# yhao-wang/DenseRetrievalToolkits

Measured on AMD Instinct MI355X. Metric: queries/sec@top-1000, 10Mx768 corpus (BASELINE: passages encoded/sec + queries/sec@top-1000, 10Mx768 corpus, 1/2/4/8 GPU), higher is better.
Workload: dtype bf16

## Files before the change

denseretrievaltoolkits_amd/_native.py:

```python
from __future__ import annotations

import ctypes
import os
import threading

import torch

from .build_native import LIB_PATH

DRT_OK = 0
DRT_EINVAL = -1
ROW_STATS_LEN = 34

_lock = threading.Lock()
_lib = None

c_i32 = ctypes.c_int32
c_i64 = ctypes.c_int64
c_sz = ctypes.c_size_t
c_vp = ctypes.c_void_p
c_f32 = ctypes.c_float
c_u64 = ctypes.c_uint64

_SIGNATURES = [
    ("drt_version", ctypes.c_char_p, []),
    ("drt_ip_topk_workspace", c_sz, [c_i64, c_i64, c_i32, c_i32]),
    ("drt_ip_topk_bf16", c_i32, [c_vp, c_i64, c_vp, c_i64, c_i32, c_i32, c_i64, c_vp, c_vp, c_vp, c_vp, c_sz, c_vp]),
    ("drt_ip_topk_resolve_workspace", c_sz, [c_i64, c_i64, c_i32]),
    ("drt_ip_topk_resolve", c_i32, [c_vp, c_i64, c_vp, c_i64, c_i32, c_i32, c_i64, c_vp, c_vp, c_vp, c_vp, c_sz,
                                    c_vp, c_vp]),
    ("drt_topk_merge", c_i32, [c_vp, c_vp, c_i64, c_i32, c_i32, c_i32, c_vp, c_vp, c_vp]),
    ("drt_ip_topk_sample_rank", c_i32, [c_i32]),
    ("drt_ip_topk_dist_workspace", c_sz, [c_i64, c_i64, c_i64, c_i32, c_i32]),
    ("drt_ip_topk_dist_sample", c_i32, [c_vp, c_i64, c_vp, c_i64, c_i64, c_i32, c_i32, c_vp, c_vp, c_sz, c_vp]),
    ("drt_ip_topk_dist_tau", c_i32, [c_vp, c_i64, c_i32, c_i32, c_vp, c_vp]),
    ("drt_ip_topk_dist_filter", c_i32, [c_vp, c_i64, c_vp, c_i64, c_i64, c_i32, c_i32, c_i64, c_vp, c_vp, c_vp,
                                        c_sz, c_vp]),
    ("drt_ip_topk_dist_filter_chunks", c_i32, [c_vp, c_i64, c_vp, c_i64, c_i64, c_i32, c_i32, c_i64, c_vp, c_vp,
                                               c_vp, c_i32, c_vp, c_sz, c_vp]),
    ("drt_ip_topk_dist_filter_lists", c_i32, [c_vp, c_i64, c_vp, c_i64, c_i64, c_i32, c_i32, c_i64, c_vp, c_i32,
                                              c_vp, c_vp, c_vp, c_sz, c_vp]),
    ("drt_ip_topk_dist_filter_lists_at", c_i32, [c_vp, c_i64, c_vp, c_i64, c_i64, c_i32, c_i32, c_i64, c_vp,
                                                 c_i32, c_i64, c_vp, c_vp, c_vp, c_sz, c_vp]),
    ("drt_topk_merge_packed", c_i32, [c_vp, c_i64, c_i32, c_i32, c_i64, c_vp, c_vp, c_vp, c_vp]),
    ("drt_topk_merge_packed_cert", c_i32, [c_vp, c_i64, c_i32, c_i32, c_i32, c_i64, c_vp, c_vp, c_vp, c_vp]),
    ("drt_topk_merge_packed_capped", c_i32, [c_vp, c_i64, c_i32, c_i32, c_i32, c_i32, c_i64, c_vp, c_vp, c_vp,
                                             c_vp]),
    ("drt_row_stats_bf16", c_i32, [c_vp, c_i64, c_i32, c_vp, c_i32, c_vp]),
    ("drt_refine_width", c_i32, [c_i32]),
    ("drt_ip_topk_exact_bf16", c_i32, [c_vp, c_i64, c_vp, c_i64, c_i32, c_i32, c_i64, c_vp, c_vp, c_vp, c_vp, c_vp,
                                       c_sz, c_vp]),
    ("drt_hit_metrics_i8", c_i32, [c_vp, c_i64, c_i64, c_vp, c_i32, c_vp, c_vp]),
    ("drt_answer_match_i32", c_i32, [c_vp, c_i32, c_vp, c_vp, c_i64, c_i64, c_i64, c_vp, c_vp, c_i32, c_i32, c_vp,
                                     c_vp, c_vp]),
# ... 121 lines not shown
```

denseretrievaltoolkits_amd/csrc/search.hip:

```cpp
#include <algorithm>
#include <cmath>
#include <vector>

#include "drt_common.h"
#include "profile.h"

namespace drt {

constexpr int kScanThreads = 256;
constexpr int kQueriesPerWG = 128;
constexpr int kHitCap = 1024;
constexpr int kCntStride = 32;

enum { SCAN_FILTER = 0, SCAN_DENSE = 1, SCAN_TOPR = 2 };
constexpr int kTopRL = 4;

struct ScanArgs {
  const __bf16* Q;
  int64_t nq;
  int64_t ldq;
  const __bf16* P;
  int64_t ldp;
  int64_t row0;
  int64_t nrows;
  int64_t rstride;
  const float* tau;
  uint32_t* counts;
  void* out;
  int64_t cap;
  int64_t exp_hits;
  uint32_t row_base;
};

__device__ __forceinline__ void glds16(const void* gsrc, uint32_t lds_addr) {
  uint32_t keep;
  asm volatile(
      "s_mov_b32 %0, m0\n\t"
      "s_mov_b32 m0, %2\n\t"
      "s_nop 0\n\t"
      "global_load_lds_dwordx4 %1, off\n\t"
      "s_mov_b32 m0, %0"
      : "=&s"(keep)
      : "v"(gsrc), "s"(lds_addr)
      : "memory");
}

__device__ __forceinline__ void glds16_nt(const void* gsrc, uint32_t lds_addr) {
// ... 448 lines not shown
__global__ __launch_bounds__(512, 1) void ip_scan16r_kernel(ScanArgs a) {
  constexpr int NW = 8;
  using C = Scan16Cfg<D, NW>;
  constexpr int PD = C::NBUF;
  __shared__ __attribute__((aligned(16))) char smem[C::LDS_BYTES];

  const int tid = threadIdx.x;
  const int wave = __builtin_amdgcn_readfirstlane(tid >> 6);
  const int lane = tid & 63;
  const int r = lane & 15;
  const int kq = lane >> 4;
  uint64_t* hk = (uint64_t*)(smem + C::HIT_KEY_OFF) + wave * kWaveSeg;
  uint8_t* hq = (uint8_t*)(smem + C::HIT_Q_OFF) + wave * kWaveSeg;

  const int64_t qbase = (int64_t)blockIdx.y * kQueriesPerWG;
  const int ntiles = (int)((a.nrows + kT16 - 1) / kT16);
  const uint32_t nrows = (uint32_t)a.nrows;
  const int t0 = blockIdx.x;
  const int tstep = gridDim.x;
  const int my_tiles = t0 < ntiles ? (ntiles - 1 - t0) / tstep + 1 : 0;
  if (my_tiles == 0) return;
  const int partial_tile = (a.nrows & (kT16 - 1)) != 0 ? ntiles - 1 : -1;
  const uint32_t ring = lds_addr_of(smem);
  const int64_t tile_stride = (int64_t)tstep * kT16 * a.ldp * 2;
  const char* next_base = (const char*)(a.P + (int64_t)t0 * kT16 * a.ldp);

  const int64_t qw = qbase + wave * 16;
  const int64_t qg = qw + r;
  const bool qok = qg < a.nq;
  const int64_t qs = qok ? qg : 0;
  bf16x8 qf[C::KS];
#pragma unroll
  for (int s = 0; s < C::KS; ++s) qf[s] = *(const bf16x8*)(a.Q + qs * a.ldq + s * 32 + kq * 8);
  float tau = __builtin_nanf("");
  {
    const float tv = a.tau[qs];
    tau = qok ? tv : tau;
  }
  if (!qok) {
#pragma unroll
    for (int s = 0; s < C::KS; ++s) qf[s] = (bf16x8){};
  }
#pragma unroll
  for (int s = 0; s < C::KS; ++s) asm volatile("" ::"v"(qf[s]));
  asm volatile("" ::"v"(tau));
  asm volatile("s_waitcnt vmcnt(0)" ::: "memory");

  LeanTile<D, NW> lt;
  lt.init(a, wave, lane);
#pragma unroll
  for (int p = 0; p < PD; ++p) {
    if (p < my_tiles) {
      const int tile = t0 + p * tstep;
      lt.template issue<NT>(a, ring + p * C::TILE_BYTES, next_base, tile == partial_tile, tile, wave, lane);
      next_base += tile_stride;
    }
  }
  if (wave >= NW / 2) __builtin_amdgcn_s_setprio(1);
  {
    const int last = my_tiles - 1 < PD - 1 ? my_tiles - 1 : PD - 1;
    wait_tiles_younger<C::GLDS_PER_WAVE>((int)last);
  }
  lds_barrier();

  const int sw = (r >> 1) & 7;
  int aoff[2];
#pragma unroll
  for (int m = 0; m < 2; ++m) aoff[m] = r * 128 + (((4 * m + kq) ^ sw) << 4);
  bf16x8 af[C::KS];
// ... 60 lines not shown
  };

  f32x4 accA, accB;
  uint32_t rbA = 0, rbB = 0;
  int buf = 0;
  auto iter = [&](int it, f32x4& acc, uint32_t& rb, const f32x4& prev, uint32_t rb_prev) {
    const int tile = t0 + it * tstep;
    if (it + PD <= my_tiles) {
      wait_vmcnt<C::GLDS_PER_WAVE * (PD - 2)>();
    } else if (it + 1 < my_tiles) {
      wait_tiles_younger<C::GLDS_PER_WAVE>(my_tiles - 1 - it - 1);
    }
    lds_barrier();
    if (it + PD < my_tiles) {
      const int ntile = tile + PD * tstep;
      lt.template issue<NT>(a, ring + buf * C::TILE_BYTES, next_base, ntile == partial_tile, ntile, wave, lane);
      next_base += tile_stride;
    }
    const int nslot = buf + 1 == C::NBUF ? 0 : buf + 1;
    mma_roll(acc, nslot);
    if (it > 0) epilogue(prev, rb_prev);
    rb = (uint32_t)tile * kT16 + 4 * kq;
    buf = nslot;
  };
  for (int it = 0; it < my_tiles; it += 2) {
    iter(it, accA, rbA, accB, rbB);
    if (it + 1 < my_tiles) iter(it + 1, accB, rbB, accA, rbA);
  }
  if (my_tiles & 1) epilogue(accA, rbA);
  else epilogue(accB, rbB);
  if (wcnt) wave_flush_hits(a, qw, hk, hq, wcnt, lane);
}

template <int D>
struct Scan32Cfg {
  static constexpr int KS = D / 32;
  static constexpr int RD = KS % 2 == 0 ? 2 : 1;
// ... 17 lines not shown
  constexpr int PD = NB - 1;
  constexpr int KS = C32::KS;
  constexpr int RD = C32::RD;
  constexpr int kSeg = kHitCap / NW;
  __shared__ __attribute__((aligned(16))) char smem[C32::LDS_BYTES];

  const int tid = threadIdx.x;
  const int wave = __builtin_amdgcn_readfirstlane(tid >> 6);
  const int lane = tid & 63;
  const int r = lane & 15;
  const int kq = lane >> 4;
  uint64_t* hk = (uint64_t*)(smem + C32::RING_BYTES) + wave * kSeg;
  uint8_t* hq = (uint8_t*)(smem + C32::RING_BYTES + kHitCap * 8) + wave * kSeg;

  const int64_t qbase = (int64_t)blockIdx.y * kQueriesPerWG32;
  const int ntiles = (int)((a.nrows + kT16 - 1) / kT16);
  const uint32_t nrows = (uint32_t)a.nrows;
  const int t0 = blockIdx.x;
  const int tstep = gridDim.x;
  const int my_tiles = t0 < ntiles ? (ntiles - 1 - t0) / tstep + 1 : 0;
  if (my_tiles == 0) return;
  const int partial_tile = (a.nrows & (kT16 - 1)) != 0 ? ntiles - 1 : -1;
  const uint32_t ring = lds_addr_of(smem);
  const int64_t tile_stride = (int64_t)tstep * kT16 * a.ldp * 2;
  const char* next_base = (const char*)(a.P + (int64_t)t0 * kT16 * a.ldp);

  const int64_t qw = qbase + wave * 32;
  bf16x8 qf0[KS], qf1[KS];
  float tau0, tau1;
  {
    const int64_t g0 = qw + r, g1 = qw + 16 + r;
    const bool ok0 = g0 < a.nq, ok1 = g1 < a.nq;
    const int64_t s0 = ok0 ? g0 : 0, s1 = ok1 ? g1 : 0;
#pragma unroll
    for (int s = 0; s < KS; ++s) {
      qf0[s] = *(const bf16x8*)(a.Q + s0 * a.ldq + s * 32 + kq * 8);
      qf1[s] = *(const bf16x8*)(a.Q + s1 * a.ldq + s * 32 + kq * 8);
    }
    const float v0 = a.tau[s0], v1 = a.tau[s1];
    tau0 = ok0 ? v0 : __builtin_nanf("");
// ... 6 lines not shown
#pragma unroll
      for (int s = 0; s < KS; ++s) qf1[s] = (bf16x8){};
    }
  }
#pragma unroll
  for (int s = 0; s < KS; ++s) asm volatile("" ::"v"(qf0[s]), "v"(qf1[s]));
  asm volatile("" ::"v"(tau0), "v"(tau1));
  asm volatile("s_waitcnt vmcnt(0)" ::: "memory");

  LeanTile<D, NW> lt;
  lt.init(a, wave, lane);
#pragma unroll
  for (int p = 0; p < PD; ++p) {
    if (p < my_tiles) {
      const int tile = t0 + p * tstep;
      lt.template issue<false>(a, ring + p * C::TILE_BYTES, next_base, tile == partial_tile, tile, wave, lane);
      next_base += tile_stride;
    }
  }
  if (wave >= NW / 2) __builtin_amdgcn_s_setprio(1);
  {
    const int last = my_tiles - 1 < PD - 1 ? my_tiles - 1 : PD - 1;
    wait_tiles_younger<C::GLDS_PER_WAVE>((int)last);
  }
  lds_barrier();

  const int sw = (r >> 1) & 7;
  int aoff[2];
#pragma unroll
  for (int m = 0; m < 2; ++m) aoff[m] = r * 128 + (((4 * m + kq) ^ sw) << 4);
  auto frag = [&](int slot, int s) -> bf16x8 {
// ... 43 lines not shown
    }
    lds_barrier();
    const bool do_dma = it + PD < my_tiles;
    const int ntile = tile + PD * tstep;
    const int pslot = buf == 0 ? NB - 1 : buf - 1;
    const int nslot = buf + 1 == NB ? 0 : buf + 1;
    acc0 = (f32x4){0.f, 0.f, 0.f, 0.f};
    acc1 = (f32x4){0.f, 0.f, 0.f, 0.f};
#pragma unroll
    for (int s = 0; s < KS; ++s) {
      acc0 = __builtin_amdgcn_mfma_f32_16x16x32_bf16(af[s % RD], qf0[s], acc0, 0, 0, 0);
      acc1 = __builtin_amdgcn_mfma_f32_16x16x32_bf16(af[s % RD], qf1[s], acc1, 0, 0, 0);
      af[s % RD] = s + RD < KS ? frag(buf, s + RD) : frag(nslot, s + RD - KS);
      __builtin_amdgcn_sched_barrier(0);
      if (s == KS / 4 && do_dma) {
        lt.template issue<false>(a, ring + pslot * C::TILE_BYTES, next_base, ntile == partial_tile, ntile, wave,
                                 lane);
        next_base += tile_stride;
      }
      __builtin_amdgcn_sched_barrier(0);
    }
    if (it > 0) epilogue(prev0, prev1, rb_prev);
    rb = (uint32_t)tile * kT16 + 4 * kq;
    buf = nslot;
  };
  f32x4 a0, a1, b0, b1;
  uint32_t rbA = 0, rbB = 0;
  for (int it = 0; it < my_tiles; it += 2) {
    iter(it, a0, a1, rbA, b0, b1, rbB);
    if (it + 1 < my_tiles) iter(it + 1, b0, b1, rbB, a0, a1, rbA);
  }
  if (my_tiles & 1) epilogue(a0, a1, rbA);
  else epilogue(b0, b1, rbB);
  if (wcnt) wave_flush_hits(a, qw, hk, hq, wcnt, lane);
}

enum { SEL_KEYS64 = 0, SEL_DENSE32 = 1 };
enum { SEL_TOPK = 0, SEL_KTH = 1 };
// ... 12 lines not shown
  int64_t n_in;
  int64_t cap;
  int64_t n_total;
  int k;
  int64_t nq;
  float* out_scores;
  int64_t* out_ids;
  int64_t ldo;
  int64_t id_offset;
  int32_t* status;
  const int32_t* qmap;
  float* tau;
  uint64_t* out_packed;
  bool global_tau;
  int k_cert;
};

template <int INPUT>
__device__ __forceinline__ uint64_t sel_load(const SelectArgs& a, int64_t q, int64_t j) {
  if (INPUT == SEL_KEYS64) return ((const uint64_t*)a.in)[q * a.in_stride + j];
  const uint32_t v = ((const uint32_t*)a.in)[q * a.in_stride + j];
  return ((uint64_t)v << 32) | (uint64_t)(uint32_t)j;
}

__device__ __forceinline__ float key_score(uint64_t x) { return desc_key_to_score((uint32_t)(x >> 32)); }

__device__ __forceinline__ int score_bin(float s, float smin, float scale) {
  if (scale == 0.0f) return 0;
  return hist_bin((s - smin) * scale, kSelBins, __builtin_signbit(s) ? 0 : kSelBins - 1);
}
// ... 409 lines not shown
  block_bitonic(buf, n2);

  const int64_t orow = a.qmap ? (int64_t)a.qmap[q] : q;
  if (a.out_packed) {
    uint64_t* op = a.out_packed + orow * (int64_t)(a.k + 1);
    for (int j = tid; j < a.k; j += kSelThreads) {
      if (j < kk_total) {
        const uint64_t x = buf[j];
        op[j] = (x & 0xFFFFFFFF00000000ull) | (uint64_t)(uint32_t)(a.id_offset + (int64_t)(x & 0xFFFFFFFFull));
      } else {
        op[j] = ~0ull;
      }
    }
    if (tid == 0) {
      const uint64_t nval = (uint64_t)(kk_total < a.k ? kk_total : a.k);
      op[a.k] = (nval << 32) | ((INPUT == SEL_KEYS64 && c_raw > a.cap) ? 1ull : 0ull) |
                (c_raw > (int64_t)a.k ? 2ull : 0ull);
    }
    return;
  }
  float* os = a.out_scores + orow * a.ldo;
  int64_t* oi = a.out_ids + orow * a.ldo;
  for (int j = tid; j < a.k; j += kSelThreads) {
    if (j < kk_total) {
      const uint64_t x = buf[j];
      os[j] = key_score(x);
      oi[j] = a.id_offset + (int64_t)(x & 0xFFFFFFFFull);
    } else {
      os[j] = kPadScore;
      oi[j] = -1;
    }
  }
  if (a.status && tid == 0) {
    int st = 0;
    if (INPUT == SEL_KEYS64) {
      if (c_raw > a.cap) st = 1;
      const int64_t kq = a.k_cert > 0 ? a.k_cert : a.k;
      if (!a.global_tau && c_raw < kq && c_raw < a.n_total) st = 1;
    }
    a.status[orow] = st;
  }
}

constexpr int kKthChunk = 4096;
constexpr int kKthThreads = 512;

__device__ __forceinline__ void block_bitonic_u32(uint32_t* buf, int n2) { block_sort<uint32_t, kKthThreads>(buf, n2); }

constexpr int kKthPer = kKthChunk / kKthThreads;
constexpr int kKthBins = 256;
constexpr int kKthSel = 1024;

__global__ __launch_bounds__(kKthThreads) void kth_partial_kernel(const uint32_t* in, int64_t stride, int64_t n,
                                                                  int r, uint32_t* part) {
  __shared__ __attribute__((aligned(16))) uint32_t buf[kKthChunk];
// ... 1717 lines not shown
static dim3 scan16_grid(int64_t nq, int64_t nrows) {
  const unsigned gy = (unsigned)((nq + kQueriesPerWG - 1) / kQueriesPerWG);
  const int64_t ntiles = (nrows + kT16 - 1) / kT16;
  int gx = scan_grid_x(ntiles);
  if (gy > 1 && ntiles >= 8) {
    const int cus = scan_grid_x((int64_t)1 << 40);
    const int share = std::max(8, (cus / (int)gy) & ~7);
    gx = (int)std::min<int64_t>(ntiles, share);
  }
  return dim3(gx, gy);
}

template <int D>
static int launch_scan_d(const ScanArgs& a, int mode, hipStream_t s) {
  if (a.nq == 0 || a.nrows == 0) return DRT_OK;
  const int64_t ntiles = (a.nrows + kT16 - 1) / kT16;
  const dim3 grid = scan16_grid(a.nq, a.nrows);
  const unsigned gy = grid.y;
  if (mode == SCAN_FILTER) {
    const double eh = a.exp_hits > 0 ? (double)a.exp_hits : (double)a.cap / 4.0;
    const bool dense_hits = eh * 256.0 / (double)a.nrows >= 0.35;
    if (D > 768 || a.row0 != 0 || a.rstride != 1) {
      if (dense_hits) hipLaunchKernelGGL((ip_scan16_kernel<D, SCAN_FILTER, 8, true>), grid, dim3(512), 0, s, a);
      else hipLaunchKernelGGL((ip_scan16_kernel<D, SCAN_FILTER, 8, false>), grid, dim3(512), 0, s, a);
    } else {
      if (D <= 768 && gy > 1) {
        const unsigned gy32 = (unsigned)((a.nq + kQueriesPerWG32 - 1) / kQueriesPerWG32);
        int gx32 = scan_grid_x(ntiles);
        if (gy32 > 1 && ntiles >= 8) {
          const int cus = scan_grid_x((int64_t)1 << 40);
          const int share = std::max(8, (cus / (int)gy32) & ~7);
          gx32 = (int)std::min<int64_t>(ntiles, share);
// ... 870 lines not shown
    a.tau = tau;
    a.counts = cnt;
    a.out = w + p.off_keys;
    a.cap = p.cap;
    a.exp_hits = p.sample ? std::max<int64_t>(1, target * rows / std::max<int64_t>(1, n_global)) : rows;
    a.row_base = (uint32_t)r0;
    const int rc = launch_scan(a, d, SCAN_FILTER, s, PROF_SCAN);
    if (rc) return rc;
  }
  sa.counts = cnt;
  sa.cap = p.cap;
  sa.n_total = n_local;
  return launch_select(sa, SEL_KEYS64, SEL_TOPK, s);
}

int drt_ip_topk_dist_filter_lists(const void* Q, int64_t nq, const void* P, int64_t n_local, int64_t n_global,
                                  int32_t d, int32_t k, int64_t id_offset, const uint32_t* lists, int32_t nlists,
                                  float* tau_out, uint64_t* packed, void* ws, size_t ws_bytes, void* stream) {
  const int32_t r = drt_ip_topk_sample_rank(k);
  return drt_ip_topk_dist_filter_lists_at(Q, nq, P, n_local, n_global, d, k, id_offset, lists, nlists,
                                          r > 0 ? nq * r : 0, tau_out, packed, ws, ws_bytes, stream);
}

int drt_ip_topk_dist_filter_lists_at(const void* Q, int64_t nq, const void* P, int64_t n_local, int64_t n_global,
                                     int32_t d, int32_t k, int64_t id_offset, const uint32_t* lists, int32_t nlists,
                                     int64_t lists_stride, float* tau_out, uint64_t* packed, void* ws,
                                     size_t ws_bytes, void* stream) {
  DRT_REQUIRE(valid_dist_dims(nq, n_local, n_global, d, k));
  DRT_REQUIRE(id_offset >= 0 && id_offset + n_local <= n_global);
  const int32_t r = drt_ip_topk_sample_rank(k);
// ... 135 lines not shown
```

denseretrievaltoolkits_amd/csrc/torch_ops.cpp:

```cpp
#include <vector>

#include <torch/library.h>
#include <ATen/ATen.h>
#include <c10/core/DeviceGuard.h>
#include <ATen/hip/impl/HIPStreamMasqueradingAsCUDA.h>

#include "drt.h"

namespace {

using at::Tensor;

void* stream_of(const Tensor& t) {
  return (void*)at::hip::getCurrentHIPStreamMasqueradingAsCUDA(t.device().index()).stream();
}

void check_rc(int rc, const char* what) {
  TORCH_CHECK_VALUE(rc != DRT_EINVAL, what, ": invalid argument (DRT_EINVAL)");
  TORCH_CHECK(rc == DRT_OK, what, ": HIP error ", rc);
}

void need_gpu(const Tensor& t, const char* name) {
  TORCH_CHECK(t.is_cuda(), "drt ops run on the GPU only (", name, " is on ", t.device(),
              "; no CPU fallback exists)");
// ... 370 lines not shown
  TORCH_CHECK_VALUE(tau.size(0) == q.size(0), "tau must hold one threshold per query");
  TORCH_CHECK_VALUE(packed.is_contiguous() && packed.size(0) == q.size(0) && packed.size(1) == k + 1,
                    "packed must be a contiguous [nq, k + 1] tensor");
  TORCH_CHECK_VALUE(starts.size() >= 2 && starts.front() == 0 && starts.back() == p.size(0),
                    "starts must run from 0 to the shard's row count");
  for (size_t c = 1; c < starts.size(); ++c) TORCH_CHECK_VALUE(starts[c - 1] <= starts[c], "starts must not decrease");
  TORCH_CHECK_VALUE(q.size(1) <= 768, "chunked filtering takes d <= 768");
  size_t wsb = 0;
  Tensor ws = dist_ws(q, p.size(0), n_global, k, &wsb);
  const std::vector<int64_t> st(starts.begin(), starts.end());
  check_rc(drt_ip_topk_dist_filter_chunks(q.data_ptr(), q.size(0), p.size(0) ? p.data_ptr() : nullptr, p.size(0),
                                          n_global, (int32_t)q.size(1), (int32_t)k, id_offset,
                                          tau.data_ptr<float>(), (uint64_t*)packed.data_ptr<int64_t>(), st.data(),
                                          (int32_t)st.size() - 1, ws.data_ptr(), wsb, stream_of(q)),
           "drt_ip_topk_dist_filter_chunks");
}

void dist_filter_lists_into(const Tensor& q_, const Tensor& p_, int64_t n_global, int64_t k, int64_t id_offset,
                            const Tensor& lists, int64_t q0, Tensor& packed) {
  need(q_, "q", at::kBFloat16, 2);
  need(p_, "p", at::kBFloat16, 2);
  need(lists, "lists", at::kInt, 3);
  need(packed, "packed", at::kLong, 2);
  const c10::DeviceGuard g(q_.device());
  const Tensor q = q_.contiguous(), p = p_.contiguous();
  TORCH_CHECK_VALUE(lists.is_contiguous(), "lists must be a contiguous [nlists, NQ, r] tensor");
  TORCH_CHECK_VALUE(q0 >= 0 && q0 + q.size(0) <= lists.size(1), "query rows [", q0, ", ", q0 + q.size(0),
                    ") outside the lists' ", lists.size(1), " rows");
  TORCH_CHECK_VALUE(packed.is_contiguous() && packed.size(0) == q.size(0) && packed.size(1) == k + 1,
                    "packed must be a contiguous [nq, k + 1] tensor");
// ... 195 lines not shown
  m.def("merge_exact(Tensor keys, Tensor ids, int k) -> (Tensor, Tensor)");
  m.def("row_stats(Tensor p, Tensor? prev=None) -> Tensor");
  m.def("refine_delta(Tensor q, Tensor p, int row_offset, Tensor cand_scores, Tensor cand_ids, int k, Tensor stats, "
        "Tensor? tau, Tensor(a!) status, bool local=False) -> (Tensor, Tensor)");
  m.def("refine_sort(Tensor cand_scores, Tensor cand_ids, Tensor delta, Tensor cnt, int k) -> (Tensor, Tensor)");
  m.def("topk_merge(Tensor scores, Tensor ids, int k_out) -> (Tensor, Tensor)");
  m.def("dist_sample(Tensor q, Tensor p, int n_global, int k) -> Tensor");
  m.def("dist_tau(Tensor lists, int k) -> Tensor");
  m.def("dist_filter(Tensor q, Tensor p, int n_global, int k, int id_offset, Tensor tau) -> Tensor");
  m.def("dist_filter_lists(Tensor q, Tensor p, int n_global, int k, int id_offset, Tensor lists) -> Tensor");
  m.def("dist_filter_lists_into(Tensor q, Tensor p, int n_global, int k, int id_offset, Tensor lists, int q0, "
        "Tensor(a!) packed) -> ()");
  m.def("dist_filter_into(Tensor q, Tensor p, int n_global, int k, int id_offset, Tensor tau, Tensor(a!) packed) -> ()");
  m.def("dist_filter_chunks_into(Tensor q, Tensor p, int n_global, int k, int id_offset, Tensor tau, int[] starts, "
        "Tensor(a!) packed) -> ()");
  m.def("merge_packed(Tensor parts, int k, int n_global, int k_cert=-1) -> (Tensor, Tensor, Tensor)");
  m.def("score_ce_fwd(Tensor q, Tensor p, int target_stride, float scale) -> (Tensor, Tensor, Tensor)");
  m.def("score_ce_bwd(Tensor grad, Tensor q, Tensor p, Tensor scores, Tensor lse, int target_stride, "
        "float scale) -> (Tensor, Tensor)");
  m.def("embed_ln(Tensor input_ids, Tensor? token_type_ids, Tensor word, Tensor pos, Tensor type, Tensor gamma, "
        "Tensor beta, float eps) -> Tensor");
  m.def("linear(Tensor x, Tensor w, Tensor? bias, Tensor? residual, bool gelu=False, bool fp32_out=False) -> Tensor");
  m.def("attention(Tensor qkv, Tensor? mask, int batch, int heads, float scale) -> Tensor");
  m.def("layernorm(Tensor x, Tensor gamma, Tensor beta, float eps) -> Tensor");
  m.def("pool(Tensor hidden, Tensor? mask, int mode) -> Tensor");
  m.def("l2_normalize(Tensor x) -> Tensor");
}

TORCH_LIBRARY_IMPL(drt, CUDA, m) {
  m.impl("ip_topk", &ip_topk);
  m.impl("ip_topk.out", &ip_topk_out);
  m.impl("dist_filter_chunks_into", &dist_filter_chunks_into);
  m.impl("ip_topk_resolve", &ip_topk_resolve);
  m.impl("ip_topk_resolve_wide", &ip_topk_resolve_wide);
  m.impl("ip_topk_large", &ip_topk_large);
  m.impl("ip_topk_large_keys", &ip_topk_large_keys);
  m.impl("merge_exact", &merge_exact);
  m.impl("row_stats", &row_stats);
  m.impl("refine_delta", &refine_delta);
  m.impl("refine_sort", &refine_sort);
  m.impl("topk_merge", &topk_merge);
  m.impl("dist_sample", &dist_sample);
  m.impl("dist_tau", &dist_tau);
  m.impl("dist_filter", &dist_filter);
  m.impl("dist_filter_lists", &dist_filter_lists);
  m.impl("dist_filter_lists_into", &dist_filter_lists_into);
  m.impl("dist_filter_into", &dist_filter_into);
// ... 11 lines not shown
```

denseretrievaltoolkits_amd/kernels.py:

```python
from __future__ import annotations

from typing import Optional, Tuple

import torch

from . import _native, ops


def _require_device(*ts: torch.Tensor) -> None:
    for t in ts:
        if not t.is_cuda:
            raise ValueError("DRT kernels run on the GPU only (got a CPU tensor; no CPU fallback exists)")


def ip_topk_workspace_bytes(nq: int, n: int, d: int, k: int) -> int:
    return int(_native.load().drt_ip_topk_workspace(nq, n, d, k))


def ip_topk(q: torch.Tensor, p: torch.Tensor, k: int, id_offset: int = 0, resolve: bool = True,
            out: Optional[Tuple[torch.Tensor, torch.Tensor]] = None,
            status: Optional[torch.Tensor] = None,
            stats: Optional[torch.Tensor] = None) -> Tuple[torch.Tensor, torch.Tensor, torch.Tensor]:
    drt = ops.load()
    _require_device(q, p)
# ... 229 lines not shown
    return ops.load().dist_filter_lists(q, p, n_global, k, id_offset, lists)


def dist_filter_into(q: torch.Tensor, p: torch.Tensor, n_global: int, k: int, id_offset: int, tau: torch.Tensor,
                     packed: torch.Tensor) -> None:
    _require_device(q, p, tau, packed)
    ops.load().dist_filter_into(q, p, n_global, k, id_offset, tau, packed)


def dist_filter_chunks_into(q: torch.Tensor, p: torch.Tensor, n_global: int, k: int, id_offset: int,
                            tau: torch.Tensor, starts, packed: torch.Tensor) -> None:
    _require_device(q, p, tau, packed)
    ops.load().dist_filter_chunks_into(q, p, n_global, k, id_offset, tau, [int(x) for x in starts], packed)


def dist_filter_lists_into(q: torch.Tensor, p: torch.Tensor, n_global: int, k: int, id_offset: int,
                           lists: torch.Tensor, q0: int, packed: torch.Tensor) -> None:
    _require_device(q, p, lists, packed)
    ops.load().dist_filter_lists_into(q, p, n_global, k, id_offset, lists, q0, packed)


def merge_packed(parts: torch.Tensor, k: int, n_global: int, k_cert: int = -1):
    _require_device(parts)
    if parts.dim() != 3 or not 2 <= parts.shape[2] <= k + 1:
        raise ValueError("merge_packed expects [nparts, nq, lcap + 1] with lcap <= k")
    return ops.load().merge_packed(parts, k, n_global, k_cert)


def exchange_cap(kc: int, nparts: int) -> int:
    if nparts <= 1 or nparts > 8:
# ... 21 lines not shown
```

denseretrievaltoolkits_amd/ops.py:

```python
from __future__ import annotations

import os
import threading

import torch

from . import _native
from ._native import ROW_STATS_LEN
from .build_native import OPS_LIB_PATH

_lock = threading.Lock()
_loaded = False


def load():
    global _loaded
    if _loaded:
        return torch.ops.drt
    with _lock:
        if _loaded:
            return torch.ops.drt
        _native.load()
        if not os.path.exists(OPS_LIB_PATH):
            raise RuntimeError(f"torch custom-op library not found at {OPS_LIB_PATH}; build it with "
# ... 74 lines not shown
    def _(q, p, n_global, k, id_offset, tau):
        return q.new_empty((q.shape[0], k + 1), dtype=torch.int64)

    @lib.register_fake("drt::dist_filter_lists")
    def _(q, p, n_global, k, id_offset, lists):
        return q.new_empty((q.shape[0], k + 1), dtype=torch.int64)

    @lib.register_fake("drt::dist_filter_into")
    def _(q, p, n_global, k, id_offset, tau, packed):
        return None

    @lib.register_fake("drt::dist_filter_chunks_into")
    def _(q, p, n_global, k, id_offset, tau, starts, packed):
        return None

    @lib.register_fake("drt::dist_filter_lists_into")
    def _(q, p, n_global, k, id_offset, lists, q0, packed):
        return None

    @lib.register_fake("drt::merge_packed")
    def _(parts, k, n_global, k_cert=-1):
        nq = parts.shape[1]
        return (parts.new_empty((nq, k), dtype=torch.float32), parts.new_empty((nq, k), dtype=torch.int64),
                parts.new_empty((nq,), dtype=torch.int32))

    @lib.register_fake("drt::score_ce_fwd")
    def _(q, p, target_stride, scale):
        return q.new_empty(()), q.new_empty((q.shape[0], p.shape[0])), q.new_empty((q.shape[0],))

    @lib.register_fake("drt::score_ce_bwd")
# ... 42 lines not shown
```

denseretrievaltoolkits_amd/search.py:

```python
from __future__ import annotations

from typing import Optional, Tuple

import numpy as np
import torch

from . import _native, comm, kernels, shards


def _as_device_bf16(x, device) -> torch.Tensor:
    if isinstance(x, np.ndarray):
        x = torch.from_numpy(np.ascontiguousarray(x))
    if not isinstance(x, torch.Tensor):
        raise TypeError(f"expected np.ndarray or torch.Tensor, got {type(x)}")
    return x.detach().to(device=device, dtype=torch.bfloat16).contiguous()


def _stage_host(*ts: torch.Tensor):
    dev = ts[0].device
    hs = [torch.empty(t.shape, dtype=t.dtype, pin_memory=True) for t in ts]
    with torch.cuda.device(dev):
        stream = torch.cuda.current_stream(dev)
        for h, t in zip(hs, ts):
            h.copy_(t, non_blocking=True)
# ... 37 lines not shown

def _pipeline(batches, enqueue, finish):
    pend = None
    for j, q in enumerate(batches):
        cur = enqueue(j, q)
        if pend is not None:
            yield finish(pend)
        pend = cur
    if pend is not None:
        yield finish(pend)


GROUP_QUERIES = 2048
GROUP_MIN_ROWS = 500_000
GROUP_CHUNK_ROWS = 1_250_000


def group_chunks(nrows: int, chunk_rows: int = None, nch: int = None):
    chunk_rows = GROUP_CHUNK_ROWS if chunk_rows is None else chunk_rows
    if nch is None:
        if chunk_rows <= 0 or nrows <= chunk_rows:
            return [(0, nrows)]
        nch = -(-nrows // chunk_rows)
    if nch <= 1:
        return [(0, nrows)]
    per = -(-nrows // nch)
    return [(min(nrows, c * per), min(nrows, (c + 1) * per)) for c in range(nch)]


def _groups(batches, cap=None):
# ... 39 lines not shown
        return comm.all_reduce_sum_(t, self.group)


def _gtau_enqueue_group(local, qs, k: int, n_global: int, offset: int, gather, to_host: bool = False,
                        stats=None, all_reduce_sum=None, id_shift: int = 0, chunks=None, world: int = 1,
                        side: _SideChannel = None):
    sizes = [q.shape[0] for q in qs]
    qg = qs[0] if len(qs) == 1 else torch.cat(qs)
    best = local.dist_sample(qg, n_global, k)
    lists = gather(best).contiguous()
    tau = kernels.dist_tau(lists, k)
    kc = kernels.refine_width(k) if stats is not None else k
    lc = kernels.exchange_cap(kc, world) if world > 1 and getattr(local, "exchange_capped", True) else kc
    if chunks is not None and len(chunks) > 1 and qg.shape[1] <= 768:
        lists = torch.empty((qg.shape[0], lc + 1), dtype=torch.int64, device=qg.device)
        starts = [a for a, _ in chunks] + [chunks[-1][1]]
        kernels.dist_filter_chunks_into(qg, local.rows, n_global, lc, offset, tau, starts, lists)
    elif chunks is not None and len(chunks) > 1:
        lists = torch.empty((len(chunks), qg.shape[0], kc + 1), dtype=torch.int64, device=qg.device)
        for c, (a, b) in enumerate(chunks):
            kernels.dist_filter_into(qg, local.rows[a:b], n_global, kc, offset + a, tau, lists[c])
    else:
        lists = torch.empty((qg.shape[0], lc + 1), dtype=torch.int64, device=qg.device)
        kernels.dist_filter_into(qg, local.rows, n_global, lc, offset, tau, lists)

    def exchange(gather, all_reduce_sum):
        allp = gather(lists)
        if lists.dim() == 3:
            allp = allp.reshape(-1, qg.shape[0], kc + 1)
        s, i, st = kernels.merge_packed(allp, kc, n_global, k_cert=k)
        if stats is not None:
            s, i = kernels.refine(qg, local.rows, offset, s, i, k, stats, tau, st, all_reduce_sum)
# ... 508 lines not shown
```

include/drt.h:

```cpp
#ifndef DRT_H_
#define DRT_H_

#include <stddef.h>
#include <stdint.h>

#ifdef __cplusplus
extern "C" {
#endif

#define DRT_OK 0
#define DRT_EINVAL (-1)
#define DRT_ROW_STATS_LEN 34

const char* drt_version(void);

size_t drt_ip_topk_workspace(int64_t nq, int64_t n, int32_t d, int32_t k);
int drt_ip_topk_bf16(const void* Q, int64_t nq, const void* P, int64_t n, int32_t d,
                     int32_t k, int64_t id_offset, float* out_scores, int64_t* out_ids,
                     int32_t* status, void* workspace, size_t workspace_bytes,
                     void* stream);

size_t drt_ip_topk_resolve_workspace(int64_t n_failed, int64_t n, int32_t d);
int drt_ip_topk_resolve(const void* Q, int64_t nq, const void* P, int64_t n, int32_t d,
                        int32_t k, int64_t id_offset, float* out_scores, int64_t* out_ids,
// ... 50 lines not shown
size_t drt_ip_topk_dist_workspace(int64_t nq, int64_t n_local, int64_t n_global, int32_t d,
                                  int32_t k);
int drt_ip_topk_dist_sample(const void* Q, int64_t nq, const void* P, int64_t n_local,
                            int64_t n_global, int32_t d, int32_t k, uint32_t* best, void* ws,
                            size_t ws_bytes, void* stream);
int drt_ip_topk_dist_tau(const uint32_t* lists, int64_t nq, int32_t nlists, int32_t k, float* tau,
                         void* stream);
int drt_ip_topk_dist_filter(const void* Q, int64_t nq, const void* P, int64_t n_local,
                            int64_t n_global, int32_t d, int32_t k, int64_t id_offset,
                            const float* tau, uint64_t* packed, void* ws, size_t ws_bytes,
                            void* stream);
int drt_ip_topk_dist_filter_chunks(const void* Q, int64_t nq, const void* P, int64_t n_local,
                                   int64_t n_global, int32_t d, int32_t k, int64_t id_offset,
                                   const float* tau, uint64_t* packed, const int64_t* starts,
                                   int32_t nchunks, void* ws, size_t ws_bytes, void* stream);
int drt_ip_topk_dist_filter_lists(const void* Q, int64_t nq, const void* P, int64_t n_local,
                                  int64_t n_global, int32_t d, int32_t k, int64_t id_offset,
                                  const uint32_t* lists, int32_t nlists, float* tau_out,
                                  uint64_t* packed, void* ws, size_t ws_bytes, void* stream);
int drt_ip_topk_dist_filter_lists_at(const void* Q, int64_t nq, const void* P, int64_t n_local,
                                     int64_t n_global, int32_t d, int32_t k, int64_t id_offset,
                                     const uint32_t* lists, int32_t nlists, int64_t lists_stride,
                                     float* tau_out, uint64_t* packed, void* ws, size_t ws_bytes,
                                     void* stream);
int drt_topk_merge_packed(const uint64_t* parts, int64_t nq, int32_t nparts, int32_t k,
                          int64_t n_global, float* out_scores, int64_t* out_ids, int32_t* status,
                          void* stream);
int drt_topk_merge_packed_capped(const uint64_t* parts, int64_t nq, int32_t nparts, int32_t lcap, int32_t k,
                                 int32_t k_cert, int64_t n_global, float* out_scores, int64_t* out_ids,
                                 int32_t* status, void* stream);
// ... 124 lines not shown
```

Measured before the change: 83690.

## Tighten filter threshold after an interleaved first scan pass

Splits the filtered corpus scan into interleaved tile passes. After the first pass, a radix-select kernel per query raises the threshold to the r-th best score seen so far, and later passes use it, so fewer candidates are emitted into the key buffer and the final select has less to sort. A certification check in the select kernel flags queries where the tightened threshold could have dropped true top-k results. The cost is extra kernel launches, a per-query histogram pass, and strided tile access in the scan.

```diff
diff --git a/denseretrievaltoolkits_amd/_native.py b/denseretrievaltoolkits_amd/_native.py
--- a/denseretrievaltoolkits_amd/_native.py
+++ b/denseretrievaltoolkits_amd/_native.py
@@ -38,6 +38,10 @@
                                         c_sz, c_vp]),
     ("drt_ip_topk_dist_filter_chunks", c_i32, [c_vp, c_i64, c_vp, c_i64, c_i64, c_i32, c_i32, c_i64, c_vp, c_vp,
                                                c_vp, c_i32, c_vp, c_sz, c_vp]),
+    ("drt_ip_topk_tighten_rank", c_i32, [c_i64, c_i32, c_i32]),
+    ("drt_ip_topk_filter_passes_workspace", c_sz, [c_i64, c_i64, c_i64, c_i32, c_i32]),
+    ("drt_ip_topk_filter_passes", c_i32, [c_vp, c_i64, c_vp, c_i64, c_i64, c_i32, c_i32, c_i64, c_vp, c_vp,
+                                          c_i32, c_i32, c_vp, c_vp, c_vp, c_sz, c_vp]),
     ("drt_ip_topk_dist_filter_lists", c_i32, [c_vp, c_i64, c_vp, c_i64, c_i64, c_i32, c_i32, c_i64, c_vp, c_i32,
                                               c_vp, c_vp, c_vp, c_sz, c_vp]),
     ("drt_ip_topk_dist_filter_lists_at", c_i32, [c_vp, c_i64, c_vp, c_i64, c_i64, c_i32, c_i32, c_i64, c_vp,
diff --git a/denseretrievaltoolkits_amd/csrc/search.hip b/denseretrievaltoolkits_amd/csrc/search.hip
--- a/denseretrievaltoolkits_amd/csrc/search.hip
+++ b/denseretrievaltoolkits_amd/csrc/search.hip
@@ -30,7 +30,13 @@
   int64_t cap;
   int64_t exp_hits;
   uint32_t row_base;
+  int32_t npass;
+  int32_t pass;
 };
+
+__host__ __device__ __forceinline__ int pass_tiles(int ntiles, int npass, int pass) {
+  return npass <= 1 ? ntiles : (pass < ntiles ? (ntiles - 1 - pass) / npass + 1 : 0);
+}
 
 __device__ __forceinline__ void glds16(const void* gsrc, uint32_t lds_addr) {
   uint32_t keep;
@@ -509,16 +515,19 @@
   uint8_t* hq = (uint8_t*)(smem + C::HIT_Q_OFF) + wave * kWaveSeg;
 
   const int64_t qbase = (int64_t)blockIdx.y * kQueriesPerWG;
-  const int ntiles = (int)((a.nrows + kT16 - 1) / kT16);
+  const int tmul = a.npass > 1 ? a.npass : 1;
+  const int tph = a.npass > 1 ? a.pass : 0;
+  const int tall = (int)((a.nrows + kT16 - 1) / kT16);
+  const int ntiles = pass_tiles(tall, a.npass, a.pass);
   const uint32_t nrows = (uint32_t)a.nrows;
   const int t0 = blockIdx.x;
   const int tstep = gridDim.x;
   const int my_tiles = t0 < ntiles ? (ntiles - 1 - t0) / tstep + 1 : 0;
   if (my_tiles == 0) return;
-  const int partial_tile = (a.nrows & (kT16 - 1)) != 0 ? ntiles - 1 : -1;
+  const int partial_tile = ((a.nrows & (kT16 - 1)) != 0 && (tall - 1) % tmul == tph) ? ntiles - 1 : -1;
   const uint32_t ring = lds_addr_of(smem);
-  const int64_t tile_stride = (int64_t)tstep * kT16 * a.ldp * 2;
-  const char* next_base = (const char*)(a.P + (int64_t)t0 * kT16 * a.ldp);
+  const int64_t tile_stride = (int64_t)tstep * tmul * kT16 * a.ldp * 2;
+  const char* next_base = (const char*)(a.P + ((int64_t)t0 * tmul + tph) * kT16 * a.ldp);
 
   const int64_t qw = qbase + wave * 16;
   const int64_t qg = qw + r;
@@ -547,7 +556,8 @@
   for (int p = 0; p < PD; ++p) {
     if (p < my_tiles) {
       const int tile = t0 + p * tstep;
-      lt.template issue<NT>(a, ring + p * C::TILE_BYTES, next_base, tile == partial_tile, tile, wave, lane);
+      lt.template issue<NT>(a, ring + p * C::TILE_BYTES, next_base, tile == partial_tile, tile * tmul + tph, wave,
+                            lane);
       next_base += tile_stride;
     }
   }
@@ -638,13 +648,14 @@
     lds_barrier();
     if (it + PD < my_tiles) {
       const int ntile = tile + PD * tstep;
-      lt.template issue<NT>(a, ring + buf * C::TILE_BYTES, next_base, ntile == partial_tile, ntile, wave, lane);
+      lt.template issue<NT>(a, ring + buf * C::TILE_BYTES, next_base, ntile == partial_tile, ntile * tmul + tph,
+                            wave, lane);
       next_base += tile_stride;
     }
     const int nslot = buf + 1 == C::NBUF ? 0 : buf + 1;
     mma_roll(acc, nslot);
     if (it > 0) epilogue(prev, rb_prev);
-    rb = (uint32_t)tile * kT16 + 4 * kq;
+    rb = (uint32_t)(tile * tmul + tph) * kT16 + 4 * kq;
     buf = nslot;
   };
   for (int it = 0; it < my_tiles; it += 2) {
@@ -692,16 +703,19 @@
   uint8_t* hq = (uint8_t*)(smem + C32::RING_BYTES + kHitCap * 8) + wave * kSeg;
 
   const int64_t qbase = (int64_t)blockIdx.y * kQueriesPerWG32;
-  const int ntiles = (int)((a.nrows + kT16 - 1) / kT16);
+  const int tmul = a.npass > 1 ? a.npass : 1;
+  const int tph = a.npass > 1 ? a.pass : 0;
+  const int tall = (int)((a.nrows + kT16 - 1) / kT16);
+  const int ntiles = pass_tiles(tall, a.npass, a.pass);
   const uint32_t nrows = (uint32_t)a.nrows;
   const int t0 = blockIdx.x;
   const int tstep = gridDim.x;
   const int my_tiles = t0 < ntiles ? (ntiles - 1 - t0) / tstep + 1 : 0;
   if (my_tiles == 0) return;
-  const int partial_tile = (a.nrows & (kT16 - 1)) != 0 ? ntiles - 1 : -1;
+  const int partial_tile = ((a.nrows & (kT16 - 1)) != 0 && (tall - 1) % tmul == tph) ? ntiles - 1 : -1;
   const uint32_t ring = lds_addr_of(smem);
-  const int64_t tile_stride = (int64_t)tstep * kT16 * a.ldp * 2;
-  const char* next_base = (const char*)(a.P + (int64_t)t0 * kT16 * a.ldp);
+  const int64_t tile_stride = (int64_t)tstep * tmul * kT16 * a.ldp * 2;
+  const char* next_base = (const char*)(a.P + ((int64_t)t0 * tmul + tph) * kT16 * a.ldp);
 
   const int64_t qw = qbase + wave * 32;
   bf16x8 qf0[KS], qf1[KS];
@@ -738,7 +752,8 @@
   for (int p = 0; p < PD; ++p) {
     if (p < my_tiles) {
       const int tile = t0 + p * tstep;
-      lt.template issue<false>(a, ring + p * C::TILE_BYTES, next_base, tile == partial_tile, tile, wave, lane);
+      lt.template issue<false>(a, ring + p * C::TILE_BYTES, next_base, tile == partial_tile, tile * tmul + tph, wave,
+                               lane);
       next_base += tile_stride;
     }
   }
@@ -812,14 +827,14 @@
       af[s % RD] = s + RD < KS ? frag(buf, s + RD) : frag(nslot, s + RD - KS);
       __builtin_amdgcn_sched_barrier(0);
       if (s == KS / 4 && do_dma) {
-        lt.template issue<false>(a, ring + pslot * C::TILE_BYTES, next_base, ntile == partial_tile, ntile, wave,
-                                 lane);
+        lt.template issue<false>(a, ring + pslot * C::TILE_BYTES, next_base, ntile == partial_tile,
+                                 ntile * tmul + tph, wave, lane);
         next_base += tile_stride;
       }
       __builtin_amdgcn_sched_barrier(0);
     }
     if (it > 0) epilogue(prev0, prev1, rb_prev);
-    rb = (uint32_t)tile * kT16 + 4 * kq;
+    rb = (uint32_t)(tile * tmul + tph) * kT16 + 4 * kq;
     buf = nslot;
   };
   f32x4 a0, a1, b0, b1;
@@ -862,6 +877,7 @@
   uint64_t* out_packed;
   bool global_tau;
   int k_cert;
+  const uint32_t* pass0;
 };
 
 template <int INPUT>
@@ -1301,8 +1317,12 @@
     }
     if (tid == 0) {
       const uint64_t nval = (uint64_t)(kk_total < a.k ? kk_total : a.k);
-      op[a.k] = (nval << 32) | ((INPUT == SEL_KEYS64 && c_raw > a.cap) ? 1ull : 0ull) |
-                (c_raw > (int64_t)a.k ? 2ull : 0ull);
+      bool bad = INPUT == SEL_KEYS64 && c_raw > a.cap;
+      if (INPUT == SEL_KEYS64 && a.pass0) {
+        const uint32_t* t = a.pass0 + q * 4;
+        if (t[2] && (int64_t)t[1] + (c_raw - (int64_t)t[0]) < (int64_t)a.k) bad = true;
+      }
+      op[a.k] = (nval << 32) | (bad ? 1ull : 0ull) | (c_raw > (int64_t)a.k ? 2ull : 0ull);
     }
     return;
   }
@@ -1326,6 +1346,84 @@
       if (!a.global_tau && c_raw < kq && c_raw < a.n_total) st = 1;
     }
     a.status[orow] = st;
+  }
+}
+
+constexpr int kTightThreads = 256;
+
+__global__ __launch_bounds__(kTightThreads) void tighten_kernel(const uint64_t* keys, int64_t cap,
+                                                                const uint32_t* counts, const float* tau0, int r,
+                                                                float* tau1, uint32_t* pass0) {
+  __shared__ uint32_t hist[256];
+  __shared__ uint32_t sh_prefix, sh_rem;
+  __shared__ uint32_t red[kTightThreads / 64];
+  const int tid = threadIdx.x;
+  const int64_t q = blockIdx.x;
+  const uint32_t c = counts[q * kCntStride];
+  const float t0 = tau0[q];
+  if (!((int64_t)c <= cap && c >= (uint32_t)r && t0 == t0)) {
+    if (tid == 0) {
+      tau1[q] = t0;
+      pass0[q * 4 + 0] = c;
+      pass0[q * 4 + 1] = c;
+      pass0[q * 4 + 2] = 0;
+      pass0[q * 4 + 3] = 0;
+    }
+    return;
+  }
+  const uint64_t* kq = keys + q * cap;
+  uint32_t prefix = 0, mask = 0, rem = (uint32_t)r;
+  for (int shift = 24; shift >= 0; shift -= 8) {
+    hist[tid] = 0;
+    __syncthreads();
+    for (uint32_t j = tid; j < c; j += kTightThreads) {
+      const uint32_t key = (uint32_t)(kq[j] >> 32);
+      if ((key & mask) == prefix) atomicAdd(&hist[(key >> shift) & 255], 1u);
+    }
+    __syncthreads();
+    if (tid < 64) {
+      const uint32_t bb[4] = {hist[4 * tid], hist[4 * tid + 1], hist[4 * tid + 2], hist[4 * tid + 3]};
+      const uint32_t s4 = bb[0] + bb[1] + bb[2] + bb[3];
+      uint32_t incl = s4;
+#pragma unroll
+      for (int o = 1; o < 64; o <<= 1) {
+        const uint32_t v = __shfl_up(incl, o, 64);
+        if (tid >= o) incl += v;
+      }
+      uint32_t run = incl - s4;
+      if (run < rem && rem <= incl) {
+        int dgt = 4 * tid;
+#pragma unroll
+        for (int t = 0; t < 3; ++t) {
+          if (dgt == 4 * tid + t && run + bb[t] < rem) {
+            run += bb[t];
+            ++dgt;
+          }
+        }
+        sh_prefix = prefix | ((uint32_t)dgt << shift);
+        sh_rem = rem - run;
+      }
+    }
+    __syncthreads();
+    prefix = sh_prefix;
+    rem = sh_rem;
+    mask |= 255u << shift;
+  }
+  const float t1 = desc_key_to_score(prefix);
+  uint32_t n = 0;
+  for (uint32_t j = tid; j < c; j += kTightThreads) n += key_score(kq[j]) >= t1 ? 1u : 0u;
+#pragma unroll
+  for (int o = 32; o > 0; o >>= 1) n += __shfl_xor(n, o, 64);
+  if ((tid & 63) == 0) red[tid >> 6] = n;
+  __syncthreads();
+  if (tid == 0) {
+    uint32_t tot = 0;
+    for (int w = 0; w < kTightThreads / 64; ++w) tot += red[w];
+    tau1[q] = t1;
+    pass0[q * 4 + 0] = c;
+    pass0[q * 4 + 1] = tot;
+    pass0[q * 4 + 2] = t1 > t0 ? 1u : 0u;
+    pass0[q * 4 + 3] = 0;
   }
 }
 
@@ -3073,8 +3171,12 @@
 template <int D>
 static int launch_scan_d(const ScanArgs& a, int mode, hipStream_t s) {
   if (a.nq == 0 || a.nrows == 0) return DRT_OK;
-  const int64_t ntiles = (a.nrows + kT16 - 1) / kT16;
-  const dim3 grid = scan16_grid(a.nq, a.nrows);
+  if (a.npass > 1 && (mode != SCAN_FILTER || D > 768 || a.row0 != 0 || a.rstride != 1 || a.pass < 0 ||
+                      a.pass >= a.npass))
+    return DRT_EINVAL;
+  const int64_t ntiles = pass_tiles((int)((a.nrows + kT16 - 1) / kT16), a.npass, a.pass);
+  if (ntiles == 0) return DRT_OK;
+  const dim3 grid = scan16_grid(a.nq, ntiles * kT16);
   const unsigned gy = grid.y;
   if (mode == SCAN_FILTER) {
     const double eh = a.exp_hits > 0 ? (double)a.exp_hits : (double)a.cap / 4.0;
@@ -3975,6 +4077,101 @@
   return launch_select(sa, SEL_KEYS64, SEL_TOPK, s);
 }
 
+int32_t drt_ip_topk_tighten_rank(int64_t n_local, int32_t npasses, int32_t k) {
+  if (n_local <= 0 || npasses <= 1 || k < 1) return 0;
+  const int64_t tall = (n_local + kT16 - 1) / kT16;
+  const int64_t t0 = (tall + npasses - 1) / npasses;
+  if (t0 >= tall) return 0;
+  const double C = (double)tall / (double)t0;
+  for (int64_t r = 1; r < ((int64_t)1 << 24); ++r) {
+    const double sigma = std::sqrt(C * (C - 1.0) * (double)r + (C - 1.0) * (double)r);
+    if (C * (double)r - 5.0 * sigma >= (double)k) return (int32_t)r;
+  }
+  return 0;
+}
+
+size_t drt_ip_topk_filter_passes_workspace(int64_t nq, int64_t n_local, int64_t n_global, int32_t d, int32_t k) {
+  if (!valid_dist_dims(nq, n_local, n_global, d, k)) return 0;
+  const TopkPlan p = make_dist_plan(nq, n_local, n_global, k);
+  return align_up(p.total, 256) + (size_t)p.nq_pad * 16;
+}
+
+int drt_ip_topk_filter_passes(const void* Q, int64_t nq, const void* P, int64_t n_local, int64_t n_global,
+                              int32_t d, int32_t k, int64_t id_offset, const float* tau, uint64_t* packed,
+                              int32_t npasses, int32_t r, float* tau1_out, uint32_t* pass0_out, void* ws,
+                              size_t ws_bytes, void* stream) {
+  DRT_REQUIRE(valid_dist_dims(nq, n_local, n_global, d, k));
+  DRT_REQUIRE(id_offset >= 0 && id_offset + n_local <= n_global);
+  DRT_REQUIRE(d <= 768 && n_local < ((int64_t)1 << 32) && npasses >= 1 && npasses <= 1024);
+  if (nq == 0) return DRT_OK;
+  DRT_REQUIRE(Q && tau && packed && ws);
+  const TopkPlan p = make_dist_plan(nq, n_local, n_global, k);
+  const size_t off_pass0 = align_up(p.total, 256);
+  DRT_REQUIRE(ws_bytes >= off_pass0 + (size_t)p.nq_pad * 16);
+  hipStream_t s = (hipStream_t)stream;
+  char* w = (char*)ws;
+  uint32_t* cnt = (uint32_t*)(w + p.off_cnt);
+  SelectArgs sa{};
+  sa.in = w + p.off_keys;
+  sa.in_stride = p.cap;
+  sa.k = k;
+  sa.nq = nq;
+  sa.id_offset = id_offset;
+  sa.out_packed = packed;
+  sa.global_tau = true;
+  if (r < 0) r = drt_ip_topk_tighten_rank(n_local, npasses, k);
+  const int tall = (int)((n_local + kT16 - 1) / kT16);
+  const bool tighten = r > 0 && n_local > 0 && pass_tiles(tall, npasses, 0) < tall;
+  if (!tighten) {
+    if (tau1_out) DRT_CHECK_HIP(hipMemcpyAsync(tau1_out, tau, (size_t)nq * 4, hipMemcpyDeviceToDevice, s));
+    if (pass0_out) DRT_CHECK_HIP(hipMemsetAsync(pass0_out, 0, (size_t)nq * 16, s));
+  }
+  if (n_local == 0) {
+    sa.n_in = 0;
+    sa.n_total = 0;
+    return launch_select(sa, SEL_DENSE32, SEL_TOPK, s);
+  }
+  DRT_REQUIRE(P != nullptr);
+  DRT_CHECK_HIP(hipMemsetAsync(cnt, 0, p.nq_pad * 4 * kCntStride, s));
+  float* tau1 = tau1_out ? tau1_out : (float*)(w + p.off_tau);
+  uint32_t* pass0 = pass0_out ? pass0_out : (uint32_t*)(w + off_pass0);
+  const int64_t target = std::max<int64_t>(4096, 4 * (int64_t)k);
+  for (int ps = 0; ps < npasses; ++ps) {
+    if (pass_tiles(tall, npasses, ps) == 0) continue;
+    ScanArgs a{};
+    a.Q = (const __bf16*)Q;
+    a.nq = nq;
+    a.ldq = d;
+    a.P = (const __bf16*)P;
+    a.ldp = d;
+    a.row0 = 0;
+    a.nrows = n_local;
+    a.rstride = 1;
+    a.tau = (tighten && ps > 0) ? tau1 : tau;
+    a.counts = cnt;
+    a.out = w + p.off_keys;
+    a.cap = p.cap;
+    a.exp_hits = p.sample ? std::max<int64_t>(1, target * n_local / npasses / std::max<int64_t>(1, n_global))
+                          : std::max<int64_t>(1, n_local / npasses);
+    a.npass = npasses;
+    a.pass = ps;
+    const int rc = launch_scan(a, d, SCAN_FILTER, s, PROF_SCAN);
+    if (rc) return rc;
+    if (tighten && ps == 0) {
+      const ProfPair pp = prof_begin(PROF_SELECT, s);
+      hipLaunchKernelGGL(tighten_kernel, dim3((unsigned)nq), dim3(kTightThreads), 0, s,
+                         (const uint64_t*)(w + p.off_keys), p.cap, (const uint32_t*)cnt, tau, (int)r, tau1, pass0);
+      prof_end(pp, s);
+      DRT_CHECK_HIP(hipGetLastError());
+    }
+  }
+  sa.counts = cnt;
+  sa.cap = p.cap;
+  sa.n_total = n_local;
+  sa.pass0 = tighten ? pass0 : nullptr;
+  return launch_select(sa, SEL_KEYS64, SEL_TOPK, s);
+}
+
 int drt_ip_topk_dist_filter_lists(const void* Q, int64_t nq, const void* P, int64_t n_local, int64_t n_global,
                                   int32_t d, int32_t k, int64_t id_offset, const uint32_t* lists, int32_t nlists,
                                   float* tau_out, uint64_t* packed, void* ws, size_t ws_bytes, void* stream) {
diff --git a/denseretrievaltoolkits_amd/csrc/torch_ops.cpp b/denseretrievaltoolkits_amd/csrc/torch_ops.cpp
--- a/denseretrievaltoolkits_amd/csrc/torch_ops.cpp
+++ b/denseretrievaltoolkits_amd/csrc/torch_ops.cpp
@@ -408,6 +408,42 @@
                                           tau.data_ptr<float>(), (uint64_t*)packed.data_ptr<int64_t>(), st.data(),
                                           (int32_t)st.size() - 1, ws.data_ptr(), wsb, stream_of(q)),
            "drt_ip_topk_dist_filter_chunks");
+}
+
+void filter_passes_into(const Tensor& q_, const Tensor& p_, int64_t n_global, int64_t k, int64_t id_offset,
+                        const Tensor& tau_, int64_t npasses, int64_t r, Tensor& packed,
+                        const c10::optional<Tensor>& tau1, const c10::optional<Tensor>& pass0) {
+  need(q_, "q", at::kBFloat16, 2);
+  need(p_, "p", at::kBFloat16, 2);
+  need(tau_, "tau", at::kFloat, 1);
+  need(packed, "packed", at::kLong, 2);
+  const c10::DeviceGuard g(q_.device());
+  const Tensor q = q_.contiguous(), p = p_.contiguous(), tau = tau_.contiguous();
+  TORCH_CHECK_VALUE(tau.size(0) == q.size(0), "tau must hold one threshold per query");
+  TORCH_CHECK_VALUE(packed.is_contiguous() && packed.size(0) == q.size(0) && packed.size(1) == k + 1,
+                    "packed must be a contiguous [nq, k + 1] tensor");
+  TORCH_CHECK_VALUE(q.size(1) <= 768, "interleaved filter passes take d <= 768");
+  TORCH_CHECK_VALUE(npasses >= 1 && npasses <= 1024, "npasses must be in [1, 1024]");
+  if (tau1.has_value()) {
+    need(*tau1, "tau1", at::kFloat, 1);
+    TORCH_CHECK_VALUE(tau1->is_contiguous() && tau1->size(0) == q.size(0), "tau1 must be a contiguous [nq] tensor");
+  }
+  if (pass0.has_value()) {
+    need(*pass0, "pass0", at::kInt, 2);
+    TORCH_CHECK_VALUE(pass0->is_contiguous() && pass0->size(0) == q.size(0) && pass0->size(1) == 4,
+                      "pass0 must be a contiguous [nq, 4] tensor");
+  }
+  const size_t wsb = drt_ip_topk_filter_passes_workspace(q.size(0), p.size(0), n_global, (int32_t)q.size(1), (int32_t)k);
+  TORCH_CHECK_VALUE(wsb > 0 || q.size(0) == 0, "unsupported dist shape nq=", q.size(0), " n_local=", p.size(0),
+                    " n_global=", n_global, " d=", q.size(1), " k=", k);
+  Tensor ws = workspace(q, wsb);
+  check_rc(drt_ip_topk_filter_passes(q.data_ptr(), q.size(0), p.size(0) ? p.data_ptr() : nullptr, p.size(0), n_global,
+                                     (int32_t)q.size(1), (int32_t)k, id_offset, tau.data_ptr<float>(),
+                                     (uint64_t*)packed.data_ptr<int64_t>(), (int32_t)npasses, (int32_t)r,
+                                     tau1.has_value() ? tau1->data_ptr<float>() : nullptr,
+                                     pass0.has_value() ? (uint32_t*)pass0->data_ptr<int32_t>() : nullptr,
+                                     ws.data_ptr(), wsb, stream_of(q)),
+           "drt_ip_topk_filter_passes");
 }
 
 void dist_filter_lists_into(const Tensor& q_, const Tensor& p_, int64_t n_global, int64_t k, int64_t id_offset,
@@ -633,6 +669,8 @@
   m.def("dist_filter_into(Tensor q, Tensor p, int n_global, int k, int id_offset, Tensor tau, Tensor(a!) packed) -> ()");
   m.def("dist_filter_chunks_into(Tensor q, Tensor p, int n_global, int k, int id_offset, Tensor tau, int[] starts, "
         "Tensor(a!) packed) -> ()");
+  m.def("filter_passes_into(Tensor q, Tensor p, int n_global, int k, int id_offset, Tensor tau, int npasses, int r, "
+        "Tensor(a!) packed, Tensor(b!)? tau1=None, Tensor(c!)? pass0=None) -> ()");
   m.def("merge_packed(Tensor parts, int k, int n_global, int k_cert=-1) -> (Tensor, Tensor, Tensor)");
   m.def("score_ce_fwd(Tensor q, Tensor p, int target_stride, float scale) -> (Tensor, Tensor, Tensor)");
   m.def("score_ce_bwd(Tensor grad, Tensor q, Tensor p, Tensor scores, Tensor lse, int target_stride, "
@@ -650,6 +688,7 @@
   m.impl("ip_topk", &ip_topk);
   m.impl("ip_topk.out", &ip_topk_out);
   m.impl("dist_filter_chunks_into", &dist_filter_chunks_into);
+  m.impl("filter_passes_into", &filter_passes_into);
   m.impl("ip_topk_resolve", &ip_topk_resolve);
   m.impl("ip_topk_resolve_wide", &ip_topk_resolve_wide);
   m.impl("ip_topk_large", &ip_topk_large);
diff --git a/denseretrievaltoolkits_amd/kernels.py b/denseretrievaltoolkits_amd/kernels.py
--- a/denseretrievaltoolkits_amd/kernels.py
+++ b/denseretrievaltoolkits_amd/kernels.py
@@ -267,6 +267,17 @@
     ops.load().dist_filter_chunks_into(q, p, n_global, k, id_offset, tau, [int(x) for x in starts], packed)
 
 
+def tighten_rank(n_local: int, npasses: int, k: int) -> int:
+    return int(_native.load().drt_ip_topk_tighten_rank(n_local, npasses, k))
+
+
+def filter_passes_into(q: torch.Tensor, p: torch.Tensor, n_global: int, k: int, id_offset: int, tau: torch.Tensor,
+                       npasses: int, packed: torch.Tensor, r: int = -1, tau1: Optional[torch.Tensor] = None,
+                       pass0: Optional[torch.Tensor] = None) -> None:
+    _require_device(q, p, tau, packed)
+    ops.load().filter_passes_into(q, p, n_global, k, id_offset, tau, npasses, r, packed, tau1, pass0)
+
+
 def dist_filter_lists_into(q: torch.Tensor, p: torch.Tensor, n_global: int, k: int, id_offset: int,
                            lists: torch.Tensor, q0: int, packed: torch.Tensor) -> None:
     _require_device(q, p, lists, packed)
diff --git a/denseretrievaltoolkits_amd/ops.py b/denseretrievaltoolkits_amd/ops.py
--- a/denseretrievaltoolkits_amd/ops.py
+++ b/denseretrievaltoolkits_amd/ops.py
@@ -112,6 +112,10 @@
     def _(q, p, n_global, k, id_offset, tau, starts, packed):
         return None
 
+    @lib.register_fake("drt::filter_passes_into")
+    def _(q, p, n_global, k, id_offset, tau, npasses, r, packed, tau1=None, pass0=None):
+        return None
+
     @lib.register_fake("drt::dist_filter_lists_into")
     def _(q, p, n_global, k, id_offset, lists, q0, packed):
         return None
diff --git a/denseretrievaltoolkits_amd/search.py b/denseretrievaltoolkits_amd/search.py
--- a/denseretrievaltoolkits_amd/search.py
+++ b/denseretrievaltoolkits_amd/search.py
@@ -75,6 +75,7 @@
 GROUP_QUERIES = 2048
 GROUP_MIN_ROWS = 500_000
 GROUP_CHUNK_ROWS = 1_250_000
+TIGHTEN_AFTER_FIRST_PASS = True
 
 
 def group_chunks(nrows: int, chunk_rows: int = None, nch: int = None):
@@ -144,8 +145,11 @@
     lc = kernels.exchange_cap(kc, world) if world > 1 and getattr(local, "exchange_capped", True) else kc
     if chunks is not None and len(chunks) > 1 and qg.shape[1] <= 768:
         lists = torch.empty((qg.shape[0], lc + 1), dtype=torch.int64, device=qg.device)
-        starts = [a for a, _ in chunks] + [chunks[-1][1]]
-        kernels.dist_filter_chunks_into(qg, local.rows, n_global, lc, offset, tau, starts, lists)
+        if TIGHTEN_AFTER_FIRST_PASS and world == 1 and offset == 0 and n_global == local.rows.shape[0]:
+            kernels.filter_passes_into(qg, local.rows, n_global, lc, offset, tau, len(chunks), lists)
+        else:
+            starts = [a for a, _ in chunks] + [chunks[-1][1]]
+            kernels.dist_filter_chunks_into(qg, local.rows, n_global, lc, offset, tau, starts, lists)
     elif chunks is not None and len(chunks) > 1:
         lists = torch.empty((len(chunks), qg.shape[0], kc + 1), dtype=torch.int64, device=qg.device)
         for c, (a, b) in enumerate(chunks):
diff --git a/include/drt.h b/include/drt.h
--- a/include/drt.h
+++ b/include/drt.h
@@ -88,6 +88,14 @@
                                    int64_t n_global, int32_t d, int32_t k, int64_t id_offset,
                                    const float* tau, uint64_t* packed, const int64_t* starts,
                                    int32_t nchunks, void* ws, size_t ws_bytes, void* stream);
+int32_t drt_ip_topk_tighten_rank(int64_t n_local, int32_t npasses, int32_t k);
+size_t drt_ip_topk_filter_passes_workspace(int64_t nq, int64_t n_local, int64_t n_global, int32_t d,
+                                           int32_t k);
+int drt_ip_topk_filter_passes(const void* Q, int64_t nq, const void* P, int64_t n_local,
+                              int64_t n_global, int32_t d, int32_t k, int64_t id_offset,
+                              const float* tau, uint64_t* packed, int32_t npasses, int32_t r,
+                              float* tau1_out, uint32_t* pass0_out, void* ws, size_t ws_bytes,
+                              void* stream);
 int drt_ip_topk_dist_filter_lists(const void* Q, int64_t nq, const void* P, int64_t n_local,
                                   int64_t n_global, int32_t d, int32_t k, int64_t id_offset,
                                   const uint32_t* lists, int32_t nlists, float* tau_out,
```

Result: faster. 85650, median of 6 (+2.3%).
